# VladimirP1/rs-sync

Hardware: AMD Instinct MI355X
Metric: ray-residuals/sec (PreSync sweep + Sync iter), 4096 frames x 2048 tracks (higher is better)
Workload: dtype f32

## Files before the change

rs-sync_amd/csrc/kernels/sync64.hpp:

```cpp
#pragma once

#pragma clang fp contract(off)

namespace {



struct Loss64Params {
    Rays64 rays;
    const FrameRec* frames;
    const uint32_t* sel;
    uint32_t n_sel;
    const d4* coef;
    int n_knots;
    double fs;
    const int32_t* kd;
    const double* fd;
    uint32_t n_delays;
    const uint32_t* grp;
    uint32_t n_grp;
    const double* M;
    const double* k;
    double* part_loss;
    double* part_grad;
    uint32_t slot0;
    const uint32_t* slots;
    uint32_t win_cap;
    uint32_t win_compact;
    uint32_t nb_run;
};

constexpr int kLossBatch = 5;
constexpr int kLossBatchWide = 3;

template <int RPT, bool GRAD, bool SIMPLE, int CAP = 0>
__global__ __launch_bounds__(kBlock, 3) void loss64_kernel(Loss64Params p) {
    constexpr int NB = GRAD ? 1 : (CAP ? kLossBatch : (RPT == 0 ? 2 : kLossBatchWide));
    d4* s_loss_win;
    uint32_t win_cap;
    if constexpr (CAP != 0) {
        __shared__ d4 s_loss_win_static[NB * 4 * CAP];
        s_loss_win = s_loss_win_static;
        win_cap = CAP;
    } else {
        extern __shared__ d4 s_loss_win_dynamic[];
        s_loss_win = s_loss_win_dynamic;
        win_cap = p.win_cap;
    }
    __shared__ double s_red[NB][2][4];
    const uint32_t nb_run = (GRAD || CAP) ? (uint32_t)NB : (p.nb_run < (uint32_t)NB ? (p.nb_run ? p.nb_run : 1u) : (uint32_t)NB);
    const int tid = threadIdx.x, lane = tid & 63, wave = tid >> 6;
    const uint32_t sf = p.slots ? p.slots[blockIdx.x] : blockIdx.x + p.slot0;
    const uint32_t g = p.grp ? p.grp[sf] : 0u;
    {
        bool any = false;
        for (uint32_t b = 0; b < p.n_delays; ++b) {
            const double f = p.fd[b * p.n_grp + g];
            any = any || f == f;
        }
        if (!any) {
            for (uint32_t b = tid; b < p.n_delays; b += kBlock) {
                p.part_loss[(size_t)b * p.n_sel + sf] = 0.0;
                if (GRAD) p.part_grad[(size_t)b * p.n_sel + sf] = 0.0;
            }
            return;
        }
    }
    const uint32_t fi = p.sel[sf];
    const FrameRec fr = p.frames[fi];
    const uint32_t N = fr.n;
    const double Mx = SIMPLE ? 0.0 : p.M[3 * sf], My = SIMPLE ? 0.0 : p.M[3 * sf + 1], Mz = SIMPLE ? 0.0 : p.M[3 * sf + 2];
    const double kk = p.k[sf];
    const d3 Mv = d3{Mx, My, Mz};
    const double inv_s = rs::loss_inv_s(SIMPLE, kk, Mv);

    for (uint32_t b0 = 0; b0 < p.n_delays; b0 += nb_run) {
        Spline64 sp[NB];
        int base[NB];
        double fdv[NB];
        bool on[NB], any_on = false;
        int kdv[NB];
#pragma unroll
        for (int q = 0; q < NB; ++q) {
            const uint32_t b = b0 + q;
            on[q] = (uint32_t)q < nb_run && b < p.n_delays;
            kdv[q] = on[q] ? p.kd[b * p.n_grp + g] : 0;
            fdv[q] = on[q] ? p.fd[b * p.n_grp + g] : 0.0;
            if (fdv[q] != fdv[q]) on[q] = false;
            any_on = any_on || on[q];
        }
        if (!any_on) {
            if ((uint32_t)tid < nb_run && b0 + tid < p.n_delays) {
                p.part_loss[(size_t)(b0 + tid) * p.n_sel + sf] = 0.0;
                if (GRAD) p.part_grad[(size_t)(b0 + tid) * p.n_sel + sf] = 0.0;
            }
            continue;
        }
        __syncthreads();
#pragma unroll
        for (int q = 0; q < NB; ++q) {
            sp[q].g = p.coef;
            sp[q].n = p.n_knots;
            sp[q].cap = (int)win_cap;
            sp[q].compact = CAP ? 0 : (int)p.win_compact;
            base[q] = fr.base_knot + kdv[q];
            if (on[q]) frame_window64<CAP>(sp[q], s_loss_win + (size_t)q * 4 * win_cap, fr, kdv[q]);
        }
        __syncthreads();
        double L[NB], G[NB];
#pragma unroll
        for (int q = 0; q < NB; ++q) L[q] = G[q] = 0.0;
        const int rpt = RPT ? RPT : (int)((N + kBlock - 1) / kBlock);
#pragma unroll 1
        for (int j = 0; j < rpt; ++j) {
            const uint32_t row = j * kBlock + tid;
            if (row < N) {
                const size_t idx = (size_t)fr.off + row;
                const double2 X = p.rays.q0[idx], Y = p.rays.q1[idx], Z = p.rays.q2[idx], T = p.rays.q3[idx];
#pragma unroll
                for (int q = 0; q < NB; ++q) {
                    if (!on[q]) continue;
                    d3 P, dP;
                    residual_row64_auto<GRAD, CAP>(sp[q], X, Y, Z, T, base[q], fdv[q], P, dP);
                    rs::loss_row<GRAD, SIMPLE>(P, dP, Mv, inv_s, L[q], G[q]);
                }
            }
        }
#pragma unroll
        for (int q = 0; q < NB; ++q) {
            const double Lw = wave_sum_f64(L[q]);
            const double Gw = GRAD ? wave_sum_f64(G[q]) : 0.0;
            if (lane == 0) {
                s_red[q][0][wave] = Lw;
                s_red[q][1][wave] = Gw;
            }
        }
        __syncthreads();
        if ((uint32_t)tid < nb_run && b0 + tid < p.n_delays) {
            const uint32_t b = b0 + tid;
            const double fdb = p.fd[b * p.n_grp + g];
            const bool live = fdb == fdb;
            const double mine = live ? s_red[tid][0][0] + s_red[tid][0][1] + s_red[tid][0][2] + s_red[tid][0][3] : 0.0;
            p.part_loss[(size_t)b * p.n_sel + sf] = mine;
            if (GRAD)
                p.part_grad[(size_t)b * p.n_sel + sf] =
                    live ? (s_red[tid][1][0] + s_red[tid][1][1] + s_red[tid][1][2] + s_red[tid][1][3]) * p.fs : 0.0;
        }
    }
}

template <int NPRE>
struct RowRays {
    double2 X[NPRE ? NPRE : 1], Y[NPRE ? NPRE : 1], Z[NPRE ? NPRE : 1], T[NPRE ? NPRE : 1];
};
template <int NPRE>
__device__ __forceinline__ void load_row_rays(const Rays64& r, const FrameRec& fr, RowRays<NPRE>& o) {
#pragma unroll
    for (int w = 0; w < NPRE; ++w) {
        const uint32_t row = (uint32_t)w * 64u + threadIdx.x;
        if (row < fr.n) {
            const size_t idx = (size_t)fr.off + row;
            o.X[w] = r.q0[idx]; o.Y[w] = r.q1[idx]; o.Z[w] = r.q2[idx]; o.T[w] = r.q3[idx];
        }
    }
}

template <bool GRAD, bool SIMPLE = false, int NPRE = 0>
__device__ __forceinline__ void loss64_wave(const Loss64Params& q, uint32_t sf, d3 Mv, double kk, int kd, double fd, d4* s_win,
                                            double& L_out, double& G_out, const RowRays<NPRE>* given = nullptr) {
    const int lane = threadIdx.x;
    const FrameRec fr = q.frames[q.sel[sf]];
    const uint32_t N = fr.n;
    const double inv_s = rs::loss_inv_s(SIMPLE, kk, Mv);
    Spline64 sp;
    sp.g = q.coef;
    sp.n = q.n_knots;
    sp.cap = (int)q.win_cap;
    sp.compact = (int)q.win_compact;
    __syncthreads();
    RowRays<NPRE> mine;
    if (NPRE && !given) load_row_rays<NPRE>(q.rays, fr, mine);
// ... 1 lines not shown
    frame_window64(sp, s_win, fr, kd);
    __syncthreads();
    const int base = fr.base_knot + kd;
    double Lw[4], Gw[4];
#pragma unroll
    for (int w = 0; w < 4; ++w) {
        Lw[w] = 0.0;
        Gw[w] = 0.0;
        if ((uint32_t)w * 64u < N) {
            double L = 0.0, G = 0.0;
            uint32_t row = (uint32_t)w * 64u + lane;
            if (w < NPRE) {
                if (row < N) {
                    d3 P, dP;
                    residual_row64_auto<GRAD>(sp, pre.X[w], pre.Y[w], pre.Z[w], pre.T[w], base, fd, P, dP);
                    rs::loss_row<GRAD, SIMPLE>(P, dP, Mv, inv_s, L, G);
                }
                row += kBlock;
            }
            for (; row < N; row += kBlock) {
                const size_t idx = (size_t)fr.off + row;
                d3 P, dP;
                residual_row64_auto<GRAD>(sp, q.rays.q0[idx], q.rays.q1[idx], q.rays.q2[idx], q.rays.q3[idx], base, fd, P, dP);
                rs::loss_row<GRAD, SIMPLE>(P, dP, Mv, inv_s, L, G);
            }
            Lw[w] = wave_sum_f64(L);
            if (GRAD) Gw[w] = wave_sum_f64(G);
        }
    }
    L_out = Lw[0] + Lw[1] + Lw[2] + Lw[3];
    G_out = GRAD ? (Gw[0] + Gw[1] + Gw[2] + Gw[3]) * q.fs : 0.0;
}

template <bool GRAD, bool SIMPLE>
__global__ __launch_bounds__(64, 3) void loss64_small_kernel(Loss64Params p) {
    extern __shared__ d4 s_win[];
    const int lane = threadIdx.x;
    const uint32_t sf = p.slots ? p.slots[blockIdx.x] : blockIdx.x + p.slot0;
    const uint32_t g = p.grp ? p.grp[sf] : 0u;
    const d3 Mv = SIMPLE ? d3{0.0, 0.0, 0.0} : d3{p.M[3 * sf], p.M[3 * sf + 1], p.M[3 * sf + 2]};
    const double kk = p.k[sf];
    for (uint32_t b = 0; b < p.n_delays; ++b) {
        const double fd = p.fd[b * p.n_grp + g];
        double Lv = 0.0, Gv = 0.0;
        if (fd == fd) loss64_wave<GRAD, SIMPLE>(p, sf, Mv, kk, p.kd[b * p.n_grp + g], fd, s_win, Lv, Gv);
        if (lane == 0) {
            p.part_loss[(size_t)b * p.n_sel + sf] = Lv;
            if (GRAD) p.part_grad[(size_t)b * p.n_sel + sf] = Gv;
        }
    }
}


struct Motion64Params {
    Rays64 rays;
    const FrameRec* frames;
    const uint32_t* sel;
    uint32_t n_sel;
    const d4* coef;
    int n_knots;
    const int32_t* kd;
    const double* fd;
    const uint32_t* grp;
    double* M;
    double* k;
    unsigned long long* stats;
    uint32_t* per_frame;
    int reeval;
    int max_iters;
    int32_t* init_h;
    uint64_t seed;
    uint32_t stream_base, stream_stride;
    const uint32_t* win_stream;
    int simple_k;
    uint32_t slot0;
    const uint32_t* order;
    uint32_t* evals_out;
    double* scratch;
    uint32_t scratch_rows;
    uint32_t scratch0;
    uint32_t win_cap;
    uint32_t win_compact;
    uint32_t win_bytes;
// ... 383 lines not shown
```

rs-sync_amd/csrc/kernels/syncloop.hpp:

```cpp
#pragma once

namespace {

constexpr int kMaxBt = 10, kHalfBt = 5;

struct SyncWin {
    double d, v;
    double x0;
    double l1, g1;
    int active, conv, hit, iters;
    int phase;
    int nf;
    int hit_prev;
};

struct SyncLoopParams {
    SyncWin* win;
    uint32_t n_win;
    uint32_t win0, win1;
    const double* part;
    uint32_t n_sel, rows;
    const uint32_t* chunk_off;
    const uint32_t* win_chunk_off;
    double* chunk_tmp;
    uint32_t chunk_stride;
    int32_t* mo_kd; double* mo_fd;
    int32_t* lg_kd; double* lg_fd;
    int32_t* tr_kd; double* tr_fd;
    double fs;
    double ts[11];
    double c_armijo, delay_b, search_center, search_radius;
    int it, max_outer;
    int nf_fixed;
    int nf_floor;
    double* ext_sums;
    int* n_active;
    double* trace;
};


__device__ __forceinline__ void split64_dev(double delay, double fs, int32_t* kd, double* fd) {
#pragma clang fp contract(off)
    if (delay != delay) { *kd = 0; *fd = delay; return; }
    const double D = delay * fs;
    const double kClamp = (double)(1 << 29);
    if (!(fabs(D) <= 1.79769313486231570e308)) { *kd = 0; *fd = 0.0; return; }
    const double fl = floor(D);
    if (fl > kClamp) { *kd = 1 << 29; *fd = 0.0; return; }
    if (fl < -kClamp) { *kd = -(1 << 29); *fd = 0.0; return; }
    *kd = (int32_t)fl;
    *fd = D - fl;
}

constexpr uint32_t kStageDoubles = 2048;
__device__ __forceinline__ void window_sums(const SyncLoopParams& p, uint32_t w, double* s_tot, double* s_stage) {
    const uint32_t c0 = p.win_chunk_off[w], c1 = p.win_chunk_off[w + 1], nc = c1 - c0;
    const uint32_t j_lo = p.chunk_off[c0], j_hi = p.chunk_off[c1], span = j_hi - j_lo;
    double* tmp = p.chunk_tmp + (size_t)w * (2 * kMaxBt) * p.chunk_stride;
    const bool staged = p.rows * span <= kStageDoubles;
    if (staged) {
        for (uint32_t e = threadIdx.x; e < p.rows * span; e += blockDim.x)
            s_stage[e] = p.part[(size_t)(e / span) * p.n_sel + j_lo + e % span];
        __syncthreads();
    }
    for (uint32_t e = threadIdx.x; e < p.rows * nc; e += blockDim.x) {
        const uint32_t r = e / nc, c = c0 + e % nc;
        double acc = 0.0;
        uint32_t j = p.chunk_off[c];
        const uint32_t j1 = p.chunk_off[c + 1];
        if (staged) {
            const double* row = s_stage + (size_t)r * span - j_lo;
            for (; j + 8 <= j1; j += 8) {
                double v[8];
#pragma unroll
                for (int q = 0; q < 8; ++q) v[q] = row[j + q];
#pragma unroll
                for (int q = 0; q < 8; ++q) acc += v[q];
            }
            for (; j < j1; ++j) acc += row[j];
        } else {
            const double* row = p.part + (size_t)r * p.n_sel;
            const uint32_t cnt = j1 - j;
            if (cnt <= 64) {
                double v[64];
#pragma unroll
                for (int q = 0; q < 64; ++q) v[q] = (uint32_t)q < cnt ? row[j + q] : 0.0;
#pragma unroll
                for (int q = 0; q < 64; ++q)
                    if ((uint32_t)q < cnt) acc += v[q];
            } else {
                for (; j < j1; ++j) acc += row[j];
            }
        }
        tmp[(size_t)r * p.chunk_stride + (c - c0)] = acc;
    }
    __syncthreads();
    for (uint32_t r = threadIdx.x; r < p.rows; r += blockDim.x) {
        const double* t = tmp + (size_t)r * p.chunk_stride;
        double acc = 0.0;
        uint32_t c = 0;
        for (; c + 16 <= nc; c += 16) {
            double v[16];
#pragma unroll
            for (int q = 0; q < 16; ++q) v[q] = t[c + q];
#pragma unroll
            for (int q = 0; q < 16; ++q) acc += v[q];
        }
        for (; c < nc; ++c) acc += t[c];
        s_tot[r] = acc;
    }
    __syncthreads();
}

__global__ __launch_bounds__(64) void sync_begin_kernel(SyncLoopParams p) {
#pragma clang fp contract(off)
    const uint32_t w = p.win0 + blockIdx.x * 64 + threadIdx.x;
    if (w >= p.win1) return;
    SyncWin& s = p.win[w];
    s.x0 = s.active ? s.d - p.delay_b * s.v : __builtin_nan("");
    split64_dev(s.active ? s.d : __builtin_nan(""), p.fs, &p.mo_kd[w], &p.mo_fd[w]);
    split64_dev(s.x0, p.fs, &p.lg_kd[w], &p.lg_fd[w]);
}
// ... 3 lines not shown
    return s.phase == 0 ? i < s.nf : i >= s.nf;
}

__device__ __forceinline__ void grad_decide(const SyncLoopParams& p, SyncWin& s, double l1, double g1) {
#pragma clang fp contract(off)
    if (s.active && s.phase == 0) {
        s.l1 = l1;
        s.g1 = g1;
        s.hit = -1;
        if (s.iters == 0 && !p.nf_fixed) {
            int i = 0;
            while (i < kMaxBt - 1 && p.ts[i] * fabs(s.g1) >= 1e-3) ++i;
            const int want = i + 2;
            s.nf = want < kHalfBt ? kHalfBt : (want > kMaxBt ? kMaxBt : want);
        }
    }
}
__device__ __forceinline__ void trial_delays(const SyncLoopParams& p, const SyncWin& s, int32_t* tr_kd, double* tr_fd, size_t stride) {
#pragma clang fp contract(off)
    for (int i = 0; i < kMaxBt; ++i) {
        const double td = trial_wanted(s, i) ? s.x0 - p.ts[i] * s.g1 : __builtin_nan("");
        split64_dev(td, p.fs, &tr_kd[(size_t)i * stride], &tr_fd[(size_t)i * stride]);
    }
}

__global__ __launch_bounds__(kBlock) void sync_sums_kernel(SyncLoopParams p) {
#pragma clang fp contract(off)
    __shared__ double s_tot[2 * kMaxBt];
    __shared__ double s_stage[kStageDoubles];
    const uint32_t w = blockIdx.x + p.win0;
    window_sums(p, w, s_tot, s_stage);
    for (uint32_t r = threadIdx.x; r < p.rows; r += blockDim.x) p.ext_sums[(size_t)r * p.n_win + w] = s_tot[r];
}
__device__ __forceinline__ void decision_sums(const SyncLoopParams& p, uint32_t w, double* s_tot, double* s_stage) {
    if (p.ext_sums) {
        for (uint32_t r = threadIdx.x; r < p.rows; r += blockDim.x) s_tot[r] = p.ext_sums[(size_t)r * p.n_win + w];
        __syncthreads();
    } else {
        window_sums(p, w, s_tot, s_stage);
    }
}

__global__ __launch_bounds__(kBlock) void sync_grad_kernel(SyncLoopParams p) {
#pragma clang fp contract(off)
    __shared__ double s_tot[2 * kMaxBt];
    __shared__ double s_stage[kStageDoubles];
    const uint32_t w = blockIdx.x + p.win0;
    decision_sums(p, w, s_tot, s_stage);
    if (threadIdx.x != 0) return;
    SyncWin& s = p.win[w];
    grad_decide(p, s, s_tot[0], s_tot[1]);
    trial_delays(p, s, p.tr_kd + w, p.tr_fd + w, p.n_win);
}

__device__ __forceinline__ void armijo(const SyncLoopParams& p, SyncWin& s, const double* lt, int b0, int b1) {
#pragma clang fp contract(off)
    if (!s.active || s.hit >= 0) return;
    const double m = s.g1 * s.g1;
    for (int i = b0; i < b1; ++i) {
        if (s.l1 - lt[i] >= p.ts[i] * p.c_armijo * m) {
            s.hit = i;
            break;
        }
    }
}

__device__ __forceinline__ bool step_decide(const SyncLoopParams& p, SyncWin& s, const double* lt, double* rows, size_t row_stride) {
#pragma clang fp contract(off)
    bool step_now = false;
    if (s.active) {
        if (s.phase == 0) {
            armijo(p, s, lt, 0, s.nf);
            if (s.hit >= 0 || s.nf >= kMaxBt) step_now = true;
            else s.phase = 1;
        } else {
            armijo(p, s, lt, s.nf, kMaxBt);
            step_now = true;
        }
    }
    if (step_now) {
        const double v = s.l1, g = s.g1;
        const double t = s.hit >= 0 ? p.ts[s.hit] : p.ts[kMaxBt];
        const int trials = s.hit >= 0 ? s.hit + 1 : kMaxBt;
        const double step = -t * g;
        s.v = p.delay_b * s.v + step;
        s.d += s.v;
        const double step_size = fabs(step);
        double* row = rows + (size_t)s.iters * row_stride;
        row[0] = s.d; row[1] = step; row[2] = v; row[3] = g; row[4] = t; row[5] = (double)trials;
        s.iters += 1;
        s.phase = 0;
        const int last = s.hit >= 0 ? s.hit : kMaxBt - 1;
        const int want = (last > s.hit_prev ? last : s.hit_prev) + 1;
        s.hit_prev = last;
        s.nf = p.nf_fixed ? p.nf_fixed : (want < p.nf_floor ? p.nf_floor : (want > kMaxBt ? kMaxBt : want));
        if (step_size < 1e-4) s.conv++; else s.conv = 0;
        bool stop = s.conv > 5;
        if (!stop && fabs(s.d - p.search_center) > p.search_radius) stop = true;
        if (stop || s.iters == p.max_outer) s.active = 0;
    }
    s.x0 = s.active ? s.d - p.delay_b * s.v : __builtin_nan("");
    return step_now;
}

__global__ __launch_bounds__(kBlock) void sync_step_kernel(SyncLoopParams p) {
#pragma clang fp contract(off)
    __shared__ double s_tot[2 * kMaxBt];
    __shared__ double s_stage[kStageDoubles];
    const uint32_t w = blockIdx.x + p.win0;
    decision_sums(p, w, s_tot, s_stage);
    if (threadIdx.x != 0) return;
    SyncWin& s = p.win[w];
    step_decide(p, s, s_tot, p.trace + (size_t)w * 6, (size_t)p.n_win * 6);
    if (s.active) atomicAdd(&p.n_active[p.it], 1);
    const bool go = s.active && s.phase == 0;
    split64_dev(go ? s.d : __builtin_nan(""), p.fs, &p.mo_kd[w], &p.mo_fd[w]);
    split64_dev(go ? s.x0 : __builtin_nan(""), p.fs, &p.lg_kd[w], &p.lg_fd[w]);
}

}
```

rs-sync_amd/csrc/rssync_kernels.hip:

```cpp
#include <hip/hip_runtime.h>

#include <dlfcn.h>

#include <algorithm>
#include <cmath>
#include <cstdio>
#include <cstdlib>
#include <cstring>
#include <mutex>
#include <string>
#include <thread>
#include <vector>

#ifndef RSSYNC_TEST_VARIANTS
#define RSSYNC_TEST_VARIANTS 0
#endif

#include "../../include/rssync_hip.h"
#include "track_hip.h"
#include "rectify_hip.h"
#include "stabilize_hip.h"
#include "device_math.hpp"
#include "sync_math.hpp"
#include "lens_math.hpp"
#include "rectify_math.hpp"
#include "stabilize_math.hpp"
#include "gyro_math.hpp"
#include "gyro_signal_math.hpp"
#include "window_plan.hpp"
#include "roctx_ranges.hpp"

using rs::f3;
using rs::f4;

#include "kernels/common.hpp"
#include "kernels/rows64.hpp"
#include "kernels/lmeds.hpp"
#include "kernels/lmeds_small.hpp"
#include "kernels/lmeds_big.hpp"
#include "kernels/support.hpp"
#include "kernels/sync64.hpp"
#include "kernels/syncloop.hpp"
#include "kernels/exec_big.hpp"
#include "kernels/executor.hpp"
#include "kernels/gyro.hpp"
#include "kernels/track.hpp"
#include "kernels/features.hpp"
#include "kernels/rectify.hpp"
#include "kernels/stabilize.hpp"


struct DevBuf {
    void* p = nullptr;
    size_t cap = 0;
};
struct TempBuf : DevBuf {
    TempBuf() = default;
    TempBuf(const TempBuf&) = delete;
    TempBuf& operator=(const TempBuf&) = delete;
    ~TempBuf() {
        if (p) (void)hipFree(p);
    }
};

constexpr int kNumClasses = 6;

struct rship_ctx {
    int device = 0;
    hipStream_t own_stream = nullptr;
    hipStream_t stream = nullptr;
    hipStream_t copy_stream = nullptr;
    hipEvent_t copy_done = nullptr;
    std::string err;
    DevBuf coef, coef64, raw, rays_a, rays_b, rays64, frames, sel, M, k, grp, grp_off, init_h;
    DevBuf pack_list, retime_ro;
// ... 537 lines not shown
            switch (rpt) {
                case 1: hipLaunchKernelGGL((lmeds_small_kernel<1, 0, 0, true>), dim3(g1), dim3(64), 0, c->stream, p); break;
                case 2: hipLaunchKernelGGL((lmeds_small_kernel<2, 0, 0, true>), dim3(g1), dim3(64), 0, c->stream, p); break;
                case 3: hipLaunchKernelGGL((lmeds_small_kernel<3, 0, 0, true>), dim3(g1), dim3(64), 0, c->stream, p); break;
                case 4: hipLaunchKernelGGL((lmeds_small_kernel<4, 0, 0, true>), dim3(g1), dim3(64), 0, c->stream, p); break;
                default: hipLaunchKernelGGL((lmeds_small_kernel<8, 0, 0, true>), dim3(g1), dim3(64), 0, c->stream, p); break;
            }
        } else {
            const uint32_t grid = (uint32_t)((uint64_t)((r.count + 7) / 8) * 8 * p.n_chunks);
            switch (rpt) {
                case 4: hipLaunchKernelGGL((lmeds_kernel<4, 0, 0, true, true>), dim3(grid), dim3(kBlock), 0, c->stream, p); break;
                case 8: hipLaunchKernelGGL((lmeds_kernel<8, 0, 0, true, true>), dim3(grid), dim3(kBlock), 0, c->stream, p); break;
                case 16: hipLaunchKernelGGL((lmeds_kernel<16, 0, 0, true, true>), dim3(grid), dim3(kBlock), 0, c->stream, p); break;
                case 24: allow_dynamic_lds(lmeds_kernel<24, 0, 0, true, true>, 0);
                         hipLaunchKernelGGL((lmeds_kernel<24, 0, 0, true, true>), dim3(grid), dim3(kBlock), 0, c->stream, p); break;
                case 32: allow_dynamic_lds(lmeds_kernel<16, 0, 0, true, true, kWideBlock>, 0);
                         hipLaunchKernelGGL((lmeds_kernel<16, 0, 0, true, true, kWideBlock>), dim3(grid), dim3(kWideBlock), 0, c->stream, p); break;
                default: return set_err(c, "lmeds (fp64 rows): unsupported rows-per-thread");
            }
        }
        RS_HIP(hipGetLastError());
    }
    return 0;
}

bool loss_fixed80(const rship_ctx* c, int k) {
    return c->cls_cap64[k] == (uint32_t)kWinMax && (class_span(c, k) + 1.f <= (float)kWinMax || c->force_general);
}
uint32_t loss_nb_run(const rship_ctx* c, int k) {
    return loss_fixed80(c, k) ? (uint32_t)kLossBatch : std::max(1u, std::min((uint32_t)kLossBatchWide, kLossWinBytes / (c->cls_cap64[k] * 128u)));
}

template <bool GRAD, bool SIMPLE>
int launch_loss64(rship_ctx* c, const Loss64Params& p_in, hipStream_t st = nullptr, uint32_t slot0 = 0, uint32_t count = 0) {
    if (!st) st = c->stream;
    ProfScope ps(c, GRAD ? RSHIP_K_LOSS_GRAD : RSHIP_K_LOSS);
    for (const ClassRange& r : class_ranges(c, slot0, count)) {
        Loss64Params p = p_in;
        const int k = r.k;
        p.slots = r.list;
        p.slot0 = r.list ? 0u : c->h_cls_slots[r.pos0];
        const uint32_t cap64 = cap64_of(c, k);
        p.win_cap = cap64;
        p.win_compact = compact_of(c, k) ? 1u : 0u;
        const bool fixed80 = !GRAD && loss_fixed80(c, k);
        p.nb_run = GRAD ? 1u : loss_nb_run(c, k);
        const size_t dyn = fixed80 ? 0 : (size_t)p.nb_run * cap64 * 128u, dyn_small = win64_bytes(c, k);
        if (k == 0 && !c->no_small_loss) {
            hipLaunchKernelGGL((loss64_small_kernel<GRAD, SIMPLE>), dim3(r.count), dim3(64), dyn_small, st, p);
            RS_HIP(hipGetLastError());
            continue;
        }
        const int rpt = k == 0 ? rpt_for(c->cls_max_n[0]) : class_rpt(c, k);
#define RS_LOSS_CASE(R)                                                                                                        \
    case R:                                                                                                                    \
        if constexpr (!GRAD) {                                                                                                 \
            if (fixed80) { hipLaunchKernelGGL((loss64_kernel<R, GRAD, SIMPLE, kWinMax>), dim3(r.count), dim3(kBlock), 0, st, p); break; } \
        }                                                                                                                      \
        hipLaunchKernelGGL((loss64_kernel<R, GRAD, SIMPLE, 0>), dim3(r.count), dim3(kBlock), dyn, st, p);                      \
        break;
        switch (rpt) {
            RS_LOSS_CASE(0)
            RS_LOSS_CASE(4)
            RS_LOSS_CASE(8)
            RS_LOSS_CASE(16)
            RS_LOSS_CASE(24)
            RS_LOSS_CASE(32)
            default: return set_err(c, "loss: unsupported rows-per-thread");
        }
#undef RS_LOSS_CASE
        RS_HIP(hipGetLastError());
    }
    return 0;
}

constexpr uint32_t kOrderMinSlots = 512;

int launch_motion64(rship_ctx* c, const Motion64Params& p_in, hipStream_t st = nullptr, uint32_t slot0 = 0, uint32_t count = 0) {
    if (!st) st = c->stream;
    ProfScope ps(c, RSHIP_K_MOTION);
    for (const ClassRange& r : class_ranges(c, slot0, count)) {
        Motion64Params p = p_in;
        const int k = r.k;
        p.slot0 = r.pos0;
        p.win_cap = cap64_of(c, k);
        p.win_compact = compact_of(c, k) ? 1u : 0u;
        const size_t dyn = win64_bytes(c, k);
        p.win_bytes = (uint32_t)dyn;
        const uint32_t cnt = r.count;
        if (k == 0) {
            const uint32_t n = c->cls_max_n[0];
            if (n <= 64) hipLaunchKernelGGL((opt_motion64_kernel<1, 1>), dim3(cnt), dim3(64), dyn, st, p);
// ... 1303 lines not shown
    if (c->prof) g = 1;
    const uint32_t by_size = n_win / 8;
    if (g > by_size) g = by_size;
    return g < 1 ? 1 : g;
}

static int sync_run_body(rship_ctx* c, const double* d0, int max_outer, double search_center, double search_radius,
                         int simplified, double* d_out, int32_t* iters, double* trace);
int rship_sync_run(rship_ctx* c, const double* d0, int max_outer, double search_center, double search_radius,
                   int simplified, double* d_out, int32_t* iters, double* trace) {
    const int rc = sync_run_body(c, d0, max_outer, search_center, search_radius, simplified, d_out, iters, trace);
    if (rc && c->rccl_comm) rccl_abort_comm(c);
    return rc;
}
static int sync_run_body(rship_ctx* c, const double* d0, int max_outer, double search_center, double search_radius,
                         int simplified, double* d_out, int32_t* iters, double* trace) {
    DeviceGuard dev_guard(c);
    const bool ranked = c->rccl_comm != nullptr || c->loop_xchg != nullptr;
    if (!c->n_knots) return set_err(c, "no gyro spline uploaded");
    if (!ranked && check_ready(c)) return 1;
    const uint32_t W = c->n_grp, ns = c->n_sel;
    if (c->plan_wins != W || c->plan_has_idx || c->plan_len != ns) return set_err(c, "sync_run: the plan must be the selection's groups");
    if (max_outer <= 0) return set_err(c, "sync_run: no iterations");
    if (c->h_grp_off.size() != (size_t)W + 1) return set_err(c, "sync_run: no selection");
    const uint32_t G = ranked ? 1u : loop_groups(c, W);
    rccl_allreduce_fn allreduce = nullptr;
    if (ranked && !c->loop_xchg && !(allreduce = (rccl_allreduce_fn)rccl_sym(c, "ncclAllReduce"))) return 1;
    std::vector<double> xbuf;
    c->loop_exchanges = 0;
    int nf_fixed = 0;
    if (const char* e = std::getenv("RSSYNC_LOOP_FIRST_TRIALS")) { const int v = atoi(e); if (v >= 1 && v <= kMaxBt) nf_fixed = v; }
    int nf_floor = (!ranked && c->max_n >= 1024u) ? 1 : kHalfBt;
    if (const char* e = std::getenv("RSSYNC_LOOP_TRIALS_FLOOR")) { const int v = atoi(e); if (v >= 1 && v <= kMaxBt) nf_floor = v; }
    const int max_launch = 2 * max_outer;
    size_t off = 0;
    auto take = [&](size_t bytes) { size_t o = off; off += (bytes + 255) / 256 * 256; return o; };
    const size_t o_win = take(W * sizeof(SyncWin));
    const size_t o_mokd = take(W * 4), o_mofd = take(W * 8), o_lgkd = take(W * 4), o_lgfd = take(W * 8);
    const size_t o_trkd = take((size_t)kMaxBt * W * 4), o_trfd = take((size_t)kMaxBt * W * 8);
    const size_t nact_stride = ((size_t)max_launch * 4 + 255) / 256 * 256;
    const size_t o_nact = take((size_t)G * nact_stride);
    const size_t o_trace = take((size_t)W * max_outer * 48);
    const size_t o_tmp = take((size_t)W * 2 * kMaxBt * (c->plan_max_chunks + 1) * 8);
    const size_t o_ext = take((size_t)2 * kMaxBt * W * 8);
    if (ensure(c, c->loop_state, off)) return 1;
    char* base = (char*)c->loop_state.p;
    if (ensure(c, c->part, (size_t)2 * kMaxBt * (ns + 1) * 8)) return 1;
    while (c->loop_streams.size() < G) {
        hipStream_t st = nullptr;
        RS_HIP(hipStreamCreateWithFlags(&st, hipStreamNonBlocking));
        c->loop_streams.push_back(st);
    }
    if (!c->loop_ready) RS_HIP(hipEventCreateWithFlags(&c->loop_ready, hipEventDisableTiming));

    std::vector<SyncWin> hw(W);
    for (uint32_t w = 0; w < W; ++w) {
        hw[w] = SyncWin{};
        hw[w].d = d0[w];
        hw[w].active = 1;
        hw[w].hit = -1;
        hw[w].nf = nf_fixed ? nf_fixed : nf_floor;
    }
    RS_HIP(hipMemcpyAsync(base + o_win, hw.data(), W * sizeof(SyncWin), hipMemcpyHostToDevice, c->stream));
    RS_HIP(hipMemsetAsync(base + o_nact, 0, (size_t)G * nact_stride, c->stream));

    SyncLoopParams lp{};
    lp.win = (SyncWin*)(base + o_win);
    lp.n_win = W;
    lp.part = (const double*)c->part.p;
    lp.n_sel = ns;
    lp.chunk_off = (const uint32_t*)c->plan_chunk_off.p;
    lp.win_chunk_off = (const uint32_t*)c->plan_win_off.p;
    lp.chunk_tmp = (double*)(base + o_tmp);
    lp.chunk_stride = c->plan_max_chunks + 1;
    lp.mo_kd = (int32_t*)(base + o_mokd); lp.mo_fd = (double*)(base + o_mofd);
    lp.lg_kd = (int32_t*)(base + o_lgkd); lp.lg_fd = (double*)(base + o_lgfd);
    lp.tr_kd = (int32_t*)(base + o_trkd); lp.tr_fd = (double*)(base + o_trfd);
    lp.fs = c->fs;
    {
        double t = 1e-3;
        for (int i = 0; i <= kMaxBt; ++i) { lp.ts[i] = t; t *= .1; }
    }
    lp.c_armijo = 2e-4;
    lp.delay_b = .3;
    lp.search_center = search_center;
    lp.search_radius = search_radius;
    lp.max_outer = max_outer;
    lp.nf_fixed = nf_fixed;
    lp.nf_floor = nf_floor;
    lp.trace = (double*)(base + o_trace);
    lp.ext_sums = ranked ? (double*)(base + o_ext) : nullptr;

    Motion64Params mp{};
    if (fill_motion(c, mp)) return 1;
    mp.kd = lp.mo_kd;
    mp.fd = lp.mo_fd;
    Loss64Params qp{};
    qp.rays = rays64_of(c);
    qp.frames = (const FrameRec*)c->frames.p;
    qp.sel = (const uint32_t*)c->sel.p;
    qp.n_sel = ns;
    qp.coef = (const d4*)c->coef64.p;
    qp.n_knots = (int)c->n_knots;
    qp.fs = c->fs;
    qp.grp = W > 1 ? (const uint32_t*)c->grp.p : nullptr;
    qp.n_grp = W;
    qp.M = (const double*)c->M.p;
    qp.k = (const double*)c->k.p;
    qp.part_loss = (double*)c->part.p;

    struct Group {
        uint32_t w0, w1, s0, s1;
        hipStream_t st;
        int* n_active;
        int* h_nact;
        int it = 0;
        bool done = false;
    };
    std::vector<Group> groups(G);
    if (ensure_pinned(c, (size_t)G * nact_stride + 64)) return 1;
    {
        uint32_t w = 0;
        for (uint32_t g = 0; g < G; ++g) {
            Group& gr = groups[g];
            gr.w0 = w;
            const uint64_t target = (uint64_t)ns * (g + 1) / G;
            while (w < W && (g + 1 == G || c->h_grp_off[w + 1] <= target || w == gr.w0)) ++w;
            if (g + 1 == G) w = W;
            gr.w1 = w;
            gr.s0 = c->h_grp_off[gr.w0];
            gr.s1 = c->h_grp_off[gr.w1];
            gr.st = G == 1 ? c->stream : c->loop_streams[g];
            gr.n_active = (int*)(base + o_nact + (size_t)g * nact_stride);
            gr.h_nact = (int*)((char*)c->pinned + (size_t)g * nact_stride);
            gr.done = gr.w1 == gr.w0;
        }
    }
    {
        std::vector<std::pair<uint32_t, uint32_t>> ranges;
        for (const Group& gr : groups)
            if (gr.s1 > gr.s0)
                for (const ClassRange& r : class_ranges(c, gr.s0, gr.s1 - gr.s0)) ranges.emplace_back(r.pos0, r.count);
        if (prepare_order(c, ranges)) return 1;
    }
    if (G > 1) {
        RS_HIP(hipEventRecord(c->loop_ready, c->stream));
        for (Group& gr : groups) RS_HIP(hipStreamWaitEvent(gr.st, c->loop_ready, 0));
    }
    auto enqueue_iteration = [&](Group& gr) -> int {
        SyncLoopParams l = lp;
        l.win0 = gr.w0; l.win1 = gr.w1;
        l.n_active = gr.n_active;
        l.it = gr.it;
        const uint32_t nw = gr.w1 - gr.w0, cnt = gr.s1 - gr.s0;
        const dim3 ctl_block(nw > 64 ? 64 : kBlock);
        Loss64Params q = qp;
        auto loss_launch = [&](bool grad) -> int {
            if (simplified) return grad ? launch_loss64<true, true>(c, q, gr.st, gr.s0, cnt) : launch_loss64<false, true>(c, q, gr.st, gr.s0, cnt);
            return grad ? launch_loss64<true, false>(c, q, gr.st, gr.s0, cnt) : launch_loss64<false, false>(c, q, gr.st, gr.s0, cnt);
        };
        if (gr.it == 0) {
            hipLaunchKernelGGL(sync_begin_kernel, dim3((nw + 63) / 64), dim3(64), 0, gr.st, l);
            RS_HIP(hipGetLastError());
        }
        if (!simplified && cnt) {
            if (launch_motion64(c, mp, gr.st, gr.s0, cnt)) return 1;
        }
        q.kd = l.lg_kd; q.fd = l.lg_fd; q.n_delays = 1;
        q.part_grad = q.part_loss + (size_t)ns;
        if (cnt && loss_launch(true)) return 1;
        l.rows = 2;
        auto exchange = [&](uint32_t rows) -> int {
            if (!ranked) return 0;
            hipLaunchKernelGGL(sync_sums_kernel, dim3(nw), ctl_block, 0, gr.st, l);
            RS_HIP(hipGetLastError());
            c->loop_exchanges += 1;
            if (c->loop_xchg) {
                xbuf.resize((size_t)rows * W);
                RS_HIP(hipMemcpyAsync(xbuf.data(), l.ext_sums, xbuf.size() * 8, hipMemcpyDeviceToHost, gr.st));
                RS_HIP(hipStreamSynchronize(gr.st));
                const int rc = c->loop_xchg(c->loop_xchg_user, xbuf.data(), xbuf.size());
                if (rc) return set_err(c, "sync_run: the loop's host exchange failed (" + std::to_string(rc) + ")");
                RS_HIP(hipMemcpyAsync(l.ext_sums, xbuf.data(), xbuf.size() * 8, hipMemcpyHostToDevice, gr.st));
                RS_HIP(hipStreamSynchronize(gr.st));
                return 0;
            }
            const int rc = allreduce(l.ext_sums, l.ext_sums, (size_t)rows * W,  8,  0, c->rccl_comm, gr.st);
            if (rc) return set_err(c, "rccl: ncclAllReduce failed (" + std::to_string(rc) + ")");
            return 0;
        };
        if (exchange(2)) return 1;
        {
            ProfScope ps(c, RSHIP_K_REDUCE);
            hipLaunchKernelGGL(sync_grad_kernel, dim3(nw), ctl_block, 0, gr.st, l);
        }
        q.kd = l.tr_kd; q.fd = l.tr_fd; q.n_delays = kMaxBt;
        q.part_grad = nullptr;
        l.rows = kMaxBt;
        if (cnt && loss_launch(false)) return 1;
        if (exchange(kMaxBt)) return 1;
        {
            ProfScope ps(c, RSHIP_K_REDUCE);
            hipLaunchKernelGGL(sync_step_kernel, dim3(nw), ctl_block, 0, gr.st, l);
        }
        RS_HIP(hipGetLastError());
        gr.it += 1;
        return 0;
    };

    const int kLook = 8;
    auto run_group = [&](Group& gr) -> int {
        DeviceGuard guard(c);
        while (!gr.done) {
            const int later = !ranked ? kLook / 2 : (c->loop_xchg ? 1 : 2);
            const int first = (ranked && c->loop_xchg) ? 1 : kLook;
            const int until = std::min(max_launch, gr.it + (gr.it == 0 ? first : later));
            while (gr.it < until)
                if (enqueue_iteration(gr)) return 1;
            RS_HIP(hipMemcpyAsync(gr.h_nact, gr.n_active, (size_t)gr.it * 4, hipMemcpyDeviceToHost, gr.st));
            RS_HIP(hipStreamSynchronize(gr.st));
            gr.done = gr.h_nact[gr.it - 1] == 0 || gr.it >= max_launch;
        }
        return 0;
    };
    {
        std::vector<std::thread> workers;
        std::vector<int> rc(G, 0);
        for (uint32_t g = 1; g < G; ++g) workers.emplace_back([&, g] { rc[g] = run_group(groups[g]); });
        rc[0] = run_group(groups[0]);
        for (std::thread& t : workers) t.join();
        for (uint32_t g = 0; g < G; ++g)
            if (rc[g]) return 1;
    }
    int it_max = 0;
// ... 1510 lines not shown
```

Baseline: 135.9 billion.

## Fuse sync grad/step decisions into loss kernels via last-block-arrives tail

Loss kernels now finish with a tail in which each block atomically increments a per-window arrival counter. The last block to arrive for a window performs the window reduction and runs the grad or step decision in place, so the separate sync_grad_kernel and sync_step_kernel launches are skipped for non-ranked groups. The window reduction also gains a configurable loads-in-flight depth to limit register pressure inside the fused kernel. The aim is to remove two launches per iteration and their serialization gaps, at the cost of atomics, fences and a serial tail in the last block of each window.

```diff
diff --git a/rs-sync_amd/csrc/kernels/sync64.hpp b/rs-sync_amd/csrc/kernels/sync64.hpp
--- a/rs-sync_amd/csrc/kernels/sync64.hpp
+++ b/rs-sync_amd/csrc/kernels/sync64.hpp
@@ -33,9 +33,115 @@
 constexpr int kLossBatch = 5;
 constexpr int kLossBatchWide = 3;
 
+template <int RPT, bool GRAD, bool SIMPLE, int CAP>
+constexpr int loss64_nb() { return GRAD ? 1 : (CAP ? kLossBatch : (RPT == 0 ? 2 : kLossBatchWide)); }
+
+template <int RPT, bool GRAD, bool SIMPLE, int CAP>
+__device__ __forceinline__ void loss64_slot(const Loss64Params& p, uint32_t sf, uint32_t g, d4* s_loss_win, uint32_t win_cap,
+                                            double (*s_red)[2][4]) {
+    constexpr int NB = loss64_nb<RPT, GRAD, SIMPLE, CAP>();
+    const uint32_t nb_run = (GRAD || CAP) ? (uint32_t)NB : (p.nb_run < (uint32_t)NB ? (p.nb_run ? p.nb_run : 1u) : (uint32_t)NB);
+    const int tid = threadIdx.x, lane = tid & 63, wave = tid >> 6;
+    {
+        bool any = false;
+        for (uint32_t b = 0; b < p.n_delays; ++b) {
+            const double f = p.fd[b * p.n_grp + g];
+            any = any || f == f;
+        }
+        if (!any) {
+            for (uint32_t b = tid; b < p.n_delays; b += kBlock) {
+                p.part_loss[(size_t)b * p.n_sel + sf] = 0.0;
+                if (GRAD) p.part_grad[(size_t)b * p.n_sel + sf] = 0.0;
+            }
+            return;
+        }
+    }
+    const uint32_t fi = p.sel[sf];
+    const FrameRec fr = p.frames[fi];
+    const uint32_t N = fr.n;
+    const double Mx = SIMPLE ? 0.0 : p.M[3 * sf], My = SIMPLE ? 0.0 : p.M[3 * sf + 1], Mz = SIMPLE ? 0.0 : p.M[3 * sf + 2];
+    const double kk = p.k[sf];
+    const d3 Mv = d3{Mx, My, Mz};
+    const double inv_s = rs::loss_inv_s(SIMPLE, kk, Mv);
+
+    for (uint32_t b0 = 0; b0 < p.n_delays; b0 += nb_run) {
+        Spline64 sp[NB];
+        int base[NB];
+        double fdv[NB];
+        bool on[NB], any_on = false;
+        int kdv[NB];
+#pragma unroll
+        for (int q = 0; q < NB; ++q) {
+            const uint32_t b = b0 + q;
+            on[q] = (uint32_t)q < nb_run && b < p.n_delays;
+            kdv[q] = on[q] ? p.kd[b * p.n_grp + g] : 0;
+            fdv[q] = on[q] ? p.fd[b * p.n_grp + g] : 0.0;
+            if (fdv[q] != fdv[q]) on[q] = false;
+            any_on = any_on || on[q];
+        }
+        if (!any_on) {
+            if ((uint32_t)tid < nb_run && b0 + tid < p.n_delays) {
+                p.part_loss[(size_t)(b0 + tid) * p.n_sel + sf] = 0.0;
+                if (GRAD) p.part_grad[(size_t)(b0 + tid) * p.n_sel + sf] = 0.0;
+            }
+            continue;
+        }
+        __syncthreads();
+#pragma unroll
+        for (int q = 0; q < NB; ++q) {
+            sp[q].g = p.coef;
+            sp[q].n = p.n_knots;
+            sp[q].cap = (int)win_cap;
+            sp[q].compact = CAP ? 0 : (int)p.win_compact;
+            base[q] = fr.base_knot + kdv[q];
+            if (on[q]) frame_window64<CAP>(sp[q], s_loss_win + (size_t)q * 4 * win_cap, fr, kdv[q]);
+        }
+        __syncthreads();
+        double L[NB], G[NB];
+#pragma unroll
+        for (int q = 0; q < NB; ++q) L[q] = G[q] = 0.0;
+        const int rpt = RPT ? RPT : (int)((N + kBlock - 1) / kBlock);
+#pragma unroll 1
+        for (int j = 0; j < rpt; ++j) {
+            const uint32_t row = j * kBlock + tid;
+            if (row < N) {
+                const size_t idx = (size_t)fr.off + row;
+                const double2 X = p.rays.q0[idx], Y = p.rays.q1[idx], Z = p.rays.q2[idx], T = p.rays.q3[idx];
+#pragma unroll
+                for (int q = 0; q < NB; ++q) {
+                    if (!on[q]) continue;
+                    d3 P, dP;
+                    residual_row64_auto<GRAD, CAP>(sp[q], X, Y, Z, T, base[q], fdv[q], P, dP);
+                    rs::loss_row<GRAD, SIMPLE>(P, dP, Mv, inv_s, L[q], G[q]);
+                }
+            }
+        }
+#pragma unroll
+        for (int q = 0; q < NB; ++q) {
+            const double Lw = wave_sum_f64(L[q]);
+            const double Gw = GRAD ? wave_sum_f64(G[q]) : 0.0;
+            if (lane == 0) {
+                s_red[q][0][wave] = Lw;
+                s_red[q][1][wave] = Gw;
+            }
+        }
+        __syncthreads();
+        if ((uint32_t)tid < nb_run && b0 + tid < p.n_delays) {
+            const uint32_t b = b0 + tid;
+            const double fdb = p.fd[b * p.n_grp + g];
+            const bool live = fdb == fdb;
+            const double mine = live ? s_red[tid][0][0] + s_red[tid][0][1] + s_red[tid][0][2] + s_red[tid][0][3] : 0.0;
+            p.part_loss[(size_t)b * p.n_sel + sf] = mine;
+            if (GRAD)
+                p.part_grad[(size_t)b * p.n_sel + sf] =
+                    live ? (s_red[tid][1][0] + s_red[tid][1][1] + s_red[tid][1][2] + s_red[tid][1][3]) * p.fs : 0.0;
+        }
+    }
+}
+
 template <int RPT, bool GRAD, bool SIMPLE, int CAP = 0>
-__global__ __launch_bounds__(kBlock, 3) void loss64_kernel(Loss64Params p) {
-    constexpr int NB = GRAD ? 1 : (CAP ? kLossBatch : (RPT == 0 ? 2 : kLossBatchWide));
+__global__ __launch_bounds__(kBlock, 3) void loss64_kernel(Loss64Params p, SyncTail tl) {
+    constexpr int NB = loss64_nb<RPT, GRAD, SIMPLE, CAP>();
     d4* s_loss_win;
     uint32_t win_cap;
     if constexpr (CAP != 0) {
@@ -47,106 +153,13 @@
         s_loss_win = s_loss_win_dynamic;
         win_cap = p.win_cap;
     }
-    __shared__ double s_red[NB][2][4];
-    const uint32_t nb_run = (GRAD || CAP) ? (uint32_t)NB : (p.nb_run < (uint32_t)NB ? (p.nb_run ? p.nb_run : 1u) : (uint32_t)NB);
-    const int tid = threadIdx.x, lane = tid & 63, wave = tid >> 6;
+    constexpr int kTailRows = GRAD ? 2 : kMaxBt;
+    static_assert(NB * 8 > kTailRows, "the tail's sums and flag live in the wave sums' array");
+    __shared__ double s_red[NB * 8];
     const uint32_t sf = p.slots ? p.slots[blockIdx.x] : blockIdx.x + p.slot0;
     const uint32_t g = p.grp ? p.grp[sf] : 0u;
-    {
-        bool any = false;
-        for (uint32_t b = 0; b < p.n_delays; ++b) {
-            const double f = p.fd[b * p.n_grp + g];
-            any = any || f == f;
-        }
-        if (!any) {
-            for (uint32_t b = tid; b < p.n_delays; b += kBlock) {
-                p.part_loss[(size_t)b * p.n_sel + sf] = 0.0;
-                if (GRAD) p.part_grad[(size_t)b * p.n_sel + sf] = 0.0;
-            }
-            return;
-        }
-    }
-    const uint32_t fi = p.sel[sf];
-    const FrameRec fr = p.frames[fi];
-    const uint32_t N = fr.n;
-    const double Mx = SIMPLE ? 0.0 : p.M[3 * sf], My = SIMPLE ? 0.0 : p.M[3 * sf + 1], Mz = SIMPLE ? 0.0 : p.M[3 * sf + 2];
-    const double kk = p.k[sf];
-    const d3 Mv = d3{Mx, My, Mz};
-    const double inv_s = rs::loss_inv_s(SIMPLE, kk, Mv);
-
-    for (uint32_t b0 = 0; b0 < p.n_delays; b0 += nb_run) {
-        Spline64 sp[NB];
-        int base[NB];
-        double fdv[NB];
-        bool on[NB], any_on = false;
-        int kdv[NB];
-#pragma unroll
-        for (int q = 0; q < NB; ++q) {
-            const uint32_t b = b0 + q;
-            on[q] = (uint32_t)q < nb_run && b < p.n_delays;
-            kdv[q] = on[q] ? p.kd[b * p.n_grp + g] : 0;
-            fdv[q] = on[q] ? p.fd[b * p.n_grp + g] : 0.0;
-            if (fdv[q] != fdv[q]) on[q] = false;
-            any_on = any_on || on[q];
-        }
-        if (!any_on) {
-            if ((uint32_t)tid < nb_run && b0 + tid < p.n_delays) {
-                p.part_loss[(size_t)(b0 + tid) * p.n_sel + sf] = 0.0;
-                if (GRAD) p.part_grad[(size_t)(b0 + tid) * p.n_sel + sf] = 0.0;
-            }
-            continue;
-        }
-        __syncthreads();
-#pragma unroll
-        for (int q = 0; q < NB; ++q) {
-            sp[q].g = p.coef;
-            sp[q].n = p.n_knots;
-            sp[q].cap = (int)win_cap;
-            sp[q].compact = CAP ? 0 : (int)p.win_compact;
-            base[q] = fr.base_knot + kdv[q];
-            if (on[q]) frame_window64<CAP>(sp[q], s_loss_win + (size_t)q * 4 * win_cap, fr, kdv[q]);
-        }
-        __syncthreads();
-        double L[NB], G[NB];
-#pragma unroll
-        for (int q = 0; q < NB; ++q) L[q] = G[q] = 0.0;
-        const int rpt = RPT ? RPT : (int)((N + kBlock - 1) / kBlock);
-#pragma unroll 1
-        for (int j = 0; j < rpt; ++j) {
-            const uint32_t row = j * kBlock + tid;
-            if (row < N) {
-                const size_t idx = (size_t)fr.off + row;
-                const double2 X = p.rays.q0[idx], Y = p.rays.q1[idx], Z = p.rays.q2[idx], T = p.rays.q3[idx];
-#pragma unroll
-                for (int q = 0; q < NB; ++q) {
-                    if (!on[q]) continue;
-                    d3 P, dP;
-                    residual_row64_auto<GRAD, CAP>(sp[q], X, Y, Z, T, base[q], fdv[q], P, dP);
-                    rs::loss_row<GRAD, SIMPLE>(P, dP, Mv, inv_s, L[q], G[q]);
-                }
-            }
-        }
-#pragma unroll
-        for (int q = 0; q < NB; ++q) {
-            const double Lw = wave_sum_f64(L[q]);
-            const double Gw = GRAD ? wave_sum_f64(G[q]) : 0.0;
-            if (lane == 0) {
-                s_red[q][0][wave] = Lw;
-                s_red[q][1][wave] = Gw;
-            }
-        }
-        __syncthreads();
-        if ((uint32_t)tid < nb_run && b0 + tid < p.n_delays) {
-            const uint32_t b = b0 + tid;
-            const double fdb = p.fd[b * p.n_grp + g];
-            const bool live = fdb == fdb;
-            const double mine = live ? s_red[tid][0][0] + s_red[tid][0][1] + s_red[tid][0][2] + s_red[tid][0][3] : 0.0;
-            p.part_loss[(size_t)b * p.n_sel + sf] = mine;
-            if (GRAD)
-                p.part_grad[(size_t)b * p.n_sel + sf] =
-                    live ? (s_red[tid][1][0] + s_red[tid][1][1] + s_red[tid][1][2] + s_red[tid][1][3]) * p.fs : 0.0;
-        }
-    }
+    loss64_slot<RPT, GRAD, SIMPLE, CAP>(p, sf, g, s_loss_win, win_cap, reinterpret_cast<double (*)[2][4]>(s_red));
+    sync_tail<GRAD>(tl, g, s_red, reinterpret_cast<uint32_t*>(s_red + kTailRows), reinterpret_cast<double*>(s_loss_win));
 }
 
 template <int NPRE>
@@ -214,8 +227,9 @@
     G_out = GRAD ? (Gw[0] + Gw[1] + Gw[2] + Gw[3]) * q.fs : 0.0;
 }
 
+constexpr uint32_t kSmallTailBytes = 256;
 template <bool GRAD, bool SIMPLE>
-__global__ __launch_bounds__(64, 3) void loss64_small_kernel(Loss64Params p) {
+__global__ __launch_bounds__(64, 3) void loss64_small_kernel(Loss64Params p, SyncTail tl) {
     extern __shared__ d4 s_win[];
     const int lane = threadIdx.x;
     const uint32_t sf = p.slots ? p.slots[blockIdx.x] : blockIdx.x + p.slot0;
@@ -231,6 +245,8 @@
             if (GRAD) p.part_grad[(size_t)b * p.n_sel + sf] = Gv;
         }
     }
+    double* s_tail = reinterpret_cast<double*>(s_win);
+    sync_tail<GRAD>(tl, g, s_tail, reinterpret_cast<uint32_t*>(s_tail + kMaxBt), s_tail + kSmallTailBytes / 8);
 }
 
 
diff --git a/rs-sync_amd/csrc/kernels/syncloop.hpp b/rs-sync_amd/csrc/kernels/syncloop.hpp
--- a/rs-sync_amd/csrc/kernels/syncloop.hpp
+++ b/rs-sync_amd/csrc/kernels/syncloop.hpp
@@ -53,11 +53,12 @@
 }
 
 constexpr uint32_t kStageDoubles = 2048;
-__device__ __forceinline__ void window_sums(const SyncLoopParams& p, uint32_t w, double* s_tot, double* s_stage) {
+template <int FLIGHT = 64>
+__device__ __forceinline__ void window_sums(const SyncLoopParams& p, uint32_t w, double* s_tot, double* s_stage, uint32_t stage_cap = kStageDoubles) {
     const uint32_t c0 = p.win_chunk_off[w], c1 = p.win_chunk_off[w + 1], nc = c1 - c0;
     const uint32_t j_lo = p.chunk_off[c0], j_hi = p.chunk_off[c1], span = j_hi - j_lo;
     double* tmp = p.chunk_tmp + (size_t)w * (2 * kMaxBt) * p.chunk_stride;
-    const bool staged = p.rows * span <= kStageDoubles;
+    const bool staged = p.rows * span <= stage_cap;
     if (staged) {
         for (uint32_t e = threadIdx.x; e < p.rows * span; e += blockDim.x)
             s_stage[e] = p.part[(size_t)(e / span) * p.n_sel + j_lo + e % span];
@@ -81,13 +82,26 @@
         } else {
             const double* row = p.part + (size_t)r * p.n_sel;
             const uint32_t cnt = j1 - j;
-            if (cnt <= 64) {
-                double v[64];
-#pragma unroll
-                for (int q = 0; q < 64; ++q) v[q] = (uint32_t)q < cnt ? row[j + q] : 0.0;
-#pragma unroll
-                for (int q = 0; q < 64; ++q)
-                    if ((uint32_t)q < cnt) acc += v[q];
+            if (FLIGHT < 64 && cnt == 64) {
+#pragma unroll 1
+                for (int q0 = 0; q0 < 64; q0 += FLIGHT) {
+                    double v[FLIGHT];
+#pragma unroll
+                    for (int q = 0; q < FLIGHT; ++q) v[q] = row[j + q0 + q];
+#pragma unroll
+                    for (int q = 0; q < FLIGHT; ++q) acc += v[q];
+                }
+            } else if (cnt <= 64) {
+                constexpr int kRagged = FLIGHT < 64 ? FLIGHT / 2 : 64;
+#pragma unroll 1
+                for (int q0 = 0; q0 < 64; q0 += kRagged) {
+                    double v[kRagged];
+#pragma unroll
+                    for (int q = 0; q < kRagged; ++q) v[q] = (uint32_t)(q0 + q) < cnt ? row[j + q0 + q] : 0.0;
+#pragma unroll
+                    for (int q = 0; q < kRagged; ++q)
+                        if ((uint32_t)(q0 + q) < cnt) acc += v[q];
+                }
             } else {
                 for (; j < j1; ++j) acc += row[j];
             }
@@ -157,25 +171,29 @@
     window_sums(p, w, s_tot, s_stage);
     for (uint32_t r = threadIdx.x; r < p.rows; r += blockDim.x) p.ext_sums[(size_t)r * p.n_win + w] = s_tot[r];
 }
-__device__ __forceinline__ void decision_sums(const SyncLoopParams& p, uint32_t w, double* s_tot, double* s_stage) {
+template <int FLIGHT = 64>
+__device__ __forceinline__ void decision_sums(const SyncLoopParams& p, uint32_t w, double* s_tot, double* s_stage, uint32_t stage_cap = kStageDoubles) {
     if (p.ext_sums) {
         for (uint32_t r = threadIdx.x; r < p.rows; r += blockDim.x) s_tot[r] = p.ext_sums[(size_t)r * p.n_win + w];
         __syncthreads();
     } else {
-        window_sums(p, w, s_tot, s_stage);
-    }
-}
-
-__global__ __launch_bounds__(kBlock) void sync_grad_kernel(SyncLoopParams p) {
-#pragma clang fp contract(off)
-    __shared__ double s_tot[2 * kMaxBt];
-    __shared__ double s_stage[kStageDoubles];
-    const uint32_t w = blockIdx.x + p.win0;
-    decision_sums(p, w, s_tot, s_stage);
+        window_sums<FLIGHT>(p, w, s_tot, s_stage, stage_cap);
+    }
+}
+
+template <int FLIGHT = 64>
+__device__ __forceinline__ void grad_decision(const SyncLoopParams& p, uint32_t w, double* s_tot, double* s_stage, uint32_t stage_cap) {
+#pragma clang fp contract(off)
+    decision_sums<FLIGHT>(p, w, s_tot, s_stage, stage_cap);
     if (threadIdx.x != 0) return;
     SyncWin& s = p.win[w];
     grad_decide(p, s, s_tot[0], s_tot[1]);
     trial_delays(p, s, p.tr_kd + w, p.tr_fd + w, p.n_win);
+}
+__global__ __launch_bounds__(kBlock) void sync_grad_kernel(SyncLoopParams p) {
+    __shared__ double s_tot[2 * kMaxBt];
+    __shared__ double s_stage[kStageDoubles];
+    grad_decision(p, blockIdx.x + p.win0, s_tot, s_stage, kStageDoubles);
 }
 
 __device__ __forceinline__ void armijo(const SyncLoopParams& p, SyncWin& s, const double* lt, int b0, int b1) {
@@ -228,12 +246,10 @@
     return step_now;
 }
 
-__global__ __launch_bounds__(kBlock) void sync_step_kernel(SyncLoopParams p) {
-#pragma clang fp contract(off)
-    __shared__ double s_tot[2 * kMaxBt];
-    __shared__ double s_stage[kStageDoubles];
-    const uint32_t w = blockIdx.x + p.win0;
-    decision_sums(p, w, s_tot, s_stage);
+template <int FLIGHT = 64>
+__device__ __forceinline__ void step_decision(const SyncLoopParams& p, uint32_t w, double* s_tot, double* s_stage, uint32_t stage_cap) {
+#pragma clang fp contract(off)
+    decision_sums<FLIGHT>(p, w, s_tot, s_stage, stage_cap);
     if (threadIdx.x != 0) return;
     SyncWin& s = p.win[w];
     step_decide(p, s, s_tot, p.trace + (size_t)w * 6, (size_t)p.n_win * 6);
@@ -242,5 +258,41 @@
     split64_dev(go ? s.d : __builtin_nan(""), p.fs, &p.mo_kd[w], &p.mo_fd[w]);
     split64_dev(go ? s.x0 : __builtin_nan(""), p.fs, &p.lg_kd[w], &p.lg_fd[w]);
 }
-
-}
+__global__ __launch_bounds__(kBlock) void sync_step_kernel(SyncLoopParams p) {
+    __shared__ double s_tot[2 * kMaxBt];
+    __shared__ double s_stage[kStageDoubles];
+    step_decision(p, blockIdx.x + p.win0, s_tot, s_stage, kStageDoubles);
+}
+
+struct SyncTail {
+    SyncLoopParams lp;
+    uint32_t* arrive;
+    uint32_t stage_cap;
+};
+
+template <bool GRAD>
+__device__ __forceinline__ void sync_tail(const SyncTail& t, uint32_t w, double* s_tot, uint32_t* s_flag, double* s_stage) {
+    if (!t.arrive) return;
+    asm volatile("s_waitcnt vmcnt(0)" ::: "memory");
+    __syncthreads();
+    if (threadIdx.x == 0) {
+        const uint32_t span = t.lp.chunk_off[t.lp.win_chunk_off[w + 1]] - t.lp.chunk_off[t.lp.win_chunk_off[w]];
+        __builtin_amdgcn_fence(__ATOMIC_RELEASE, "agent");
+        asm volatile("s_waitcnt vmcnt(0)" ::: "memory");
+        const uint32_t before = __hip_atomic_fetch_add(&t.arrive[w], 1u, __ATOMIC_RELAXED, __HIP_MEMORY_SCOPE_AGENT);
+        const uint32_t last = before + 1u == span ? 1u : 0u;
+        if (last) {
+            __builtin_amdgcn_fence(__ATOMIC_ACQUIRE, "agent");
+            asm volatile("s_waitcnt vmcnt(0)" ::: "memory");
+        }
+        *s_flag = last;
+    }
+    __syncthreads();
+    if (!*s_flag) return;
+    __syncthreads();
+    if (GRAD) grad_decision<32>(t.lp, w, s_tot, s_stage, t.stage_cap);
+    else step_decision<32>(t.lp, w, s_tot, s_stage, t.stage_cap);
+    if (threadIdx.x == 0) __hip_atomic_store(&t.arrive[w], 0u, __ATOMIC_RELAXED, __HIP_MEMORY_SCOPE_AGENT);
+}
+
+}
diff --git a/rs-sync_amd/csrc/rssync_kernels.hip b/rs-sync_amd/csrc/rssync_kernels.hip
--- a/rs-sync_amd/csrc/rssync_kernels.hip
+++ b/rs-sync_amd/csrc/rssync_kernels.hip
@@ -39,8 +39,8 @@
 #include "kernels/lmeds_small.hpp"
 #include "kernels/lmeds_big.hpp"
 #include "kernels/support.hpp"
+#include "kernels/syncloop.hpp"
 #include "kernels/sync64.hpp"
-#include "kernels/syncloop.hpp"
 #include "kernels/exec_big.hpp"
 #include "kernels/executor.hpp"
 #include "kernels/gyro.hpp"
@@ -644,11 +644,15 @@
 }
 
 template <bool GRAD, bool SIMPLE>
-int launch_loss64(rship_ctx* c, const Loss64Params& p_in, hipStream_t st = nullptr, uint32_t slot0 = 0, uint32_t count = 0) {
+int launch_loss64(rship_ctx* c, const Loss64Params& p_in, hipStream_t st = nullptr, uint32_t slot0 = 0, uint32_t count = 0,
+                  const SyncTail* tail = nullptr) {
     if (!st) st = c->stream;
     ProfScope ps(c, GRAD ? RSHIP_K_LOSS_GRAD : RSHIP_K_LOSS);
     for (const ClassRange& r : class_ranges(c, slot0, count)) {
         Loss64Params p = p_in;
+        SyncTail tl{};
+        if (tail) tl = *tail;
+        auto stage_doubles = [](size_t bytes) { return (uint32_t)std::min<size_t>(bytes / 8, kStageDoubles); };
         const int k = r.k;
         p.slots = r.list;
         p.slot0 = r.list ? 0u : c->h_cls_slots[r.pos0];
@@ -659,17 +663,20 @@
         p.nb_run = GRAD ? 1u : loss_nb_run(c, k);
         const size_t dyn = fixed80 ? 0 : (size_t)p.nb_run * cap64 * 128u, dyn_small = win64_bytes(c, k);
         if (k == 0 && !c->no_small_loss) {
-            hipLaunchKernelGGL((loss64_small_kernel<GRAD, SIMPLE>), dim3(r.count), dim3(64), dyn_small, st, p);
+            const size_t dyn_tail = tail ? std::max(dyn_small, (size_t)2 * kSmallTailBytes) : dyn_small;
+            tl.stage_cap = stage_doubles(dyn_tail - kSmallTailBytes);
+            hipLaunchKernelGGL((loss64_small_kernel<GRAD, SIMPLE>), dim3(r.count), dim3(64), dyn_tail, st, p, tl);
             RS_HIP(hipGetLastError());
             continue;
         }
         const int rpt = k == 0 ? rpt_for(c->cls_max_n[0]) : class_rpt(c, k);
+        tl.stage_cap = stage_doubles(fixed80 ? (size_t)kLossBatch * kWinMax * 128u : dyn);
 #define RS_LOSS_CASE(R)                                                                                                        \
     case R:                                                                                                                    \
         if constexpr (!GRAD) {                                                                                                 \
-            if (fixed80) { hipLaunchKernelGGL((loss64_kernel<R, GRAD, SIMPLE, kWinMax>), dim3(r.count), dim3(kBlock), 0, st, p); break; } \
+            if (fixed80) { hipLaunchKernelGGL((loss64_kernel<R, GRAD, SIMPLE, kWinMax>), dim3(r.count), dim3(kBlock), 0, st, p, tl); break; } \
         }                                                                                                                      \
-        hipLaunchKernelGGL((loss64_kernel<R, GRAD, SIMPLE, 0>), dim3(r.count), dim3(kBlock), dyn, st, p);                      \
+        hipLaunchKernelGGL((loss64_kernel<R, GRAD, SIMPLE, 0>), dim3(r.count), dim3(kBlock), dyn, st, p, tl);                  \
         break;
         switch (rpt) {
             RS_LOSS_CASE(0)
@@ -2039,6 +2046,10 @@
     if (const char* e = std::getenv("RSSYNC_LOOP_FIRST_TRIALS")) { const int v = atoi(e); if (v >= 1 && v <= kMaxBt) nf_fixed = v; }
     int nf_floor = (!ranked && c->max_n >= 1024u) ? 1 : kHalfBt;
     if (const char* e = std::getenv("RSSYNC_LOOP_TRIALS_FLOOR")) { const int v = atoi(e); if (v >= 1 && v <= kMaxBt) nf_floor = v; }
+    bool loop_tail = true;
+#if RSSYNC_TEST_VARIANTS
+    if (const char* e = std::getenv("RSSYNC_LOOP_TAIL")) loop_tail = !(e[0] == '0' && !e[1]);
+#endif
     const int max_launch = 2 * max_outer;
     size_t off = 0;
     auto take = [&](size_t bytes) { size_t o = off; off += (bytes + 255) / 256 * 256; return o; };
@@ -2047,6 +2058,7 @@
     const size_t o_trkd = take((size_t)kMaxBt * W * 4), o_trfd = take((size_t)kMaxBt * W * 8);
     const size_t nact_stride = ((size_t)max_launch * 4 + 255) / 256 * 256;
     const size_t o_nact = take((size_t)G * nact_stride);
+    const size_t o_arrive = take((size_t)W * 4);
     const size_t o_trace = take((size_t)W * max_outer * 48);
     const size_t o_tmp = take((size_t)W * 2 * kMaxBt * (c->plan_max_chunks + 1) * 8);
     const size_t o_ext = take((size_t)2 * kMaxBt * W * 8);
@@ -2069,7 +2081,7 @@
         hw[w].nf = nf_fixed ? nf_fixed : nf_floor;
     }
     RS_HIP(hipMemcpyAsync(base + o_win, hw.data(), W * sizeof(SyncWin), hipMemcpyHostToDevice, c->stream));
-    RS_HIP(hipMemsetAsync(base + o_nact, 0, (size_t)G * nact_stride, c->stream));
+    RS_HIP(hipMemsetAsync(base + o_nact, 0, o_arrive + ((size_t)W * 4 + 255) / 256 * 256 - o_nact, c->stream));
 
     SyncLoopParams lp{};
     lp.win = (SyncWin*)(base + o_win);
@@ -2123,6 +2135,7 @@
         int* h_nact;
         int it = 0;
         bool done = false;
+        bool tail = false;
     };
     std::vector<Group> groups(G);
     if (ensure_pinned(c, (size_t)G * nact_stride + 64)) return 1;
@@ -2141,6 +2154,8 @@
             gr.n_active = (int*)(base + o_nact + (size_t)g * nact_stride);
             gr.h_nact = (int*)((char*)c->pinned + (size_t)g * nact_stride);
             gr.done = gr.w1 == gr.w0;
+            gr.tail = !ranked && loop_tail && gr.s1 > gr.s0;
+            for (uint32_t v = gr.w0; v < gr.w1 && gr.tail; ++v) gr.tail = c->h_grp_off[v + 1] > c->h_grp_off[v];
         }
     }
     {
@@ -2162,9 +2177,16 @@
         const uint32_t nw = gr.w1 - gr.w0, cnt = gr.s1 - gr.s0;
         const dim3 ctl_block(nw > 64 ? 64 : kBlock);
         Loss64Params q = qp;
+        SyncTail tl{};
         auto loss_launch = [&](bool grad) -> int {
-            if (simplified) return grad ? launch_loss64<true, true>(c, q, gr.st, gr.s0, cnt) : launch_loss64<false, true>(c, q, gr.st, gr.s0, cnt);
-            return grad ? launch_loss64<true, false>(c, q, gr.st, gr.s0, cnt) : launch_loss64<false, false>(c, q, gr.st, gr.s0, cnt);
+            const SyncTail* t = nullptr;
+            if (gr.tail) {
+                tl.lp = l;
+                tl.arrive = (uint32_t*)(base + o_arrive);
+                t = &tl;
+            }
+            if (simplified) return grad ? launch_loss64<true, true>(c, q, gr.st, gr.s0, cnt, t) : launch_loss64<false, true>(c, q, gr.st, gr.s0, cnt, t);
+            return grad ? launch_loss64<true, false>(c, q, gr.st, gr.s0, cnt, t) : launch_loss64<false, false>(c, q, gr.st, gr.s0, cnt, t);
         };
         if (gr.it == 0) {
             hipLaunchKernelGGL(sync_begin_kernel, dim3((nw + 63) / 64), dim3(64), 0, gr.st, l);
@@ -2175,8 +2197,8 @@
         }
         q.kd = l.lg_kd; q.fd = l.lg_fd; q.n_delays = 1;
         q.part_grad = q.part_loss + (size_t)ns;
+        l.rows = 2;
         if (cnt && loss_launch(true)) return 1;
-        l.rows = 2;
         auto exchange = [&](uint32_t rows) -> int {
             if (!ranked) return 0;
             hipLaunchKernelGGL(sync_sums_kernel, dim3(nw), ctl_block, 0, gr.st, l);
@@ -2197,7 +2219,7 @@
             return 0;
         };
         if (exchange(2)) return 1;
-        {
+        if (!gr.tail) {
             ProfScope ps(c, RSHIP_K_REDUCE);
             hipLaunchKernelGGL(sync_grad_kernel, dim3(nw), ctl_block, 0, gr.st, l);
         }
@@ -2206,7 +2228,7 @@
         l.rows = kMaxBt;
         if (cnt && loss_launch(false)) return 1;
         if (exchange(kMaxBt)) return 1;
-        {
+        if (!gr.tail) {
             ProfScope ps(c, RSHIP_K_REDUCE);
             hipLaunchKernelGGL(sync_step_kernel, dim3(nw), ctl_block, 0, gr.st, l);
         }
```

Measured after the change: 133.0 billion. -2.1%, worse.
